# mbdriscoll/indigo

Measured on AMD Instinct MI355X. Metric: SENSE AHA evals/sec (256^3 x 8-coil non-Cartesian), higher is better.
Workload: dtype complex64 (f32)

## Files before the change

indigo_amd/csrc/ig_spmm.hip:

```cpp
#include "ig_spmm_common.h"
#include <hip/amd_detail/amd_hip_unsafe_atomics.h>
#include <algorithm>
#include <atomic>
#include <cstring>

namespace {

struct GridMask {
    const uint32_t* bits;
    int64_t n0, nm;
};

constexpr int WL_SUB = 32;
struct WorkLists {
    int32_t*  rows[2];
    uint32_t* count;
    uint32_t  cap;
    const int32_t* yperm;
};

__device__ __forceinline__ bool wl_append(const WorkLists& wl, int which, int sub, bool want, int32_t row) {
    const uint64_t bal = __ballot(want);
    if (!bal) return false;
    const int lane = threadIdx.x & 63;
    const int leader = __ffsll((long long)bal) - 1;
    uint32_t base = 0;
    if (lane == leader) base = atomicAdd(&wl.count[which * WL_SUB + sub], (uint32_t)__popcll(bal));
    base = __shfl(base, leader, 64);
    if (!want) return false;
    const uint32_t idx = base + (uint32_t)__popcll(bal & ((1ull << lane) - 1ull));
    if (idx >= wl.cap) return false;
    wl.rows[which][(size_t)sub * wl.cap + idx] = row;
    return true;
}

__device__ __forceinline__ int64_t out_row(const int32_t* __restrict__ perm, int64_t row) {
    return perm ? (int64_t)perm[row] : row;
}

template <bool CONJ>
__device__ __forceinline__ void acc_nz(float2& acc, float2 v, float2 x) {
    if (CONJ) acc = cadd(acc, cmulc(v, x));
    else      cfma(acc, v, x);
}

template <int CL, int NL, bool CONJ, int BMODE>
__global__ void __launch_bounds__(BLK)
k_csrmm_gather(int64_t M, int64_t N,
               const int32_t* __restrict__ rowptr, const int32_t* __restrict__ colind,
               const float2* __restrict__ vals,
               const float2* __restrict__ X, int64_t ldx, int64_t sxr,
               float2* __restrict__ Y, int64_t ldy,
               float2 alpha, float2 beta, int xcd_remap,
               WorkLists wl, int32_t thr_mid, int32_t thr_long) {
    constexpr int RPW = 64 / (CL * NL);
    const int lane = threadIdx.x & 63;
    const int c = lane % CL;
    const int i = (lane / CL) % NL;
    const int r = lane / (CL * NL);
    const int64_t blk = xcd_remap ? xcd_block(blockIdx.x, gridDim.x) : (int64_t)blockIdx.x;
    const int64_t wave = blk * WAVES_PER_BLOCK + (threadIdx.x >> 6);
    const int64_t row = wave * RPW + r;
    const bool row_ok = row < M;

    int32_t p0 = 0, p1 = 0;
    if (row_ok) { p0 = rowptr[row]; p1 = rowptr[row + 1]; }

    int deferred = 0;
    const int32_t len = p1 - p0;
    {
        const int sub = (int)(wave & (WL_SUB - 1));
        const bool head = c == 0 && i == 0;
        if (wl_append(wl, 0, sub, head && len > thr_mid && len <= thr_long, (int32_t)row)) deferred = 1;
        if (wl_append(wl, 1, sub, head && len > thr_long, (int32_t)row)) deferred = 1;
    }
    deferred = __shfl(deferred, r * CL * NL, 64);
    if (deferred) p1 = p0;

    for (int64_t jb = 0; jb < N; jb += CL) {
        const int64_t j = jb + c;
        const bool col_ok = j < N;
        const float2* __restrict__ xcol = X + (col_ok ? j : 0) * ldx;
        float2 acc = make_float2(0.f, 0.f);
        for (int32_t p = p0 + i; p < p1; p += 4 * NL) {
            int32_t k4[4];
            float2 v4[4], x4[4];
#pragma unroll
            for (int u = 0; u < 4; ++u) {
                const int32_t pu = p + u * NL;
                const bool ok = pu < p1;
                const int32_t q = ok ? pu : p1 - 1;
                k4[u] = colind[q];
                const float2 vv = vals[q];
                v4[u] = ok ? vv : make_float2(0.f, 0.f);
            }
#pragma unroll
            for (int u = 0; u < 4; ++u) x4[u] = xcol[k4[u] * sxr];
#pragma unroll
            for (int u = 0; u < 4; ++u) acc_nz<CONJ>(acc, v4[u], x4[u]);
        }
#pragma unroll
        for (int off = CL * NL / 2; off >= CL; off >>= 1) {
            acc.x += __shfl_xor(acc.x, off, 64);
            acc.y += __shfl_xor(acc.y, off, 64);
        }
        if (i == 0 && row_ok && col_ok && !deferred) {
            float2* yp = Y + j * ldy + out_row(wl.yperm, row);
            float2 out = cmul(alpha, acc);
            if (BMODE == 1) cfma(out, beta, *yp);
            *yp = out;
        }
    }
}

template <int VW, int CLV, int NL, bool CONJ, int BMODE, bool REALW = false>
__global__ void __launch_bounds__(BLK)
k_csrmm_gather_v(int64_t M, const int32_t* __restrict__ rowptr, const int32_t* __restrict__ colind,
                 const float2* __restrict__ vals, const float2* __restrict__ X, int64_t sxr,
                 float2* __restrict__ Y, int64_t ldy, float2 alpha, float2 beta, int xcd_remap,
                 WorkLists wl, int32_t thr_mid, int32_t thr_long) {
    static_assert(VW % 2 == 0 && CLV * NL <= 64, "16-byte loads; a row's lanes fit a wave");
    constexpr int LPR = CLV * NL, RPW = 64 / LPR, NV = VW / 2;
    const int lane = threadIdx.x & 63;
    const int c = lane % CLV, i = (lane / CLV) % NL, r = lane / LPR;
    const int64_t blk = xcd_remap ? xcd_block(blockIdx.x, gridDim.x) : (int64_t)blockIdx.x;
    const int64_t wave = blk * WAVES_PER_BLOCK + (threadIdx.x >> 6);
    const int64_t row = wave * RPW + r;
    const bool row_ok = row < M;
    int32_t p0 = 0, p1 = 0;
    if (row_ok) { p0 = rowptr[row]; p1 = rowptr[row + 1]; }
    int deferred = 0;
    const int32_t len = p1 - p0;
    {
        const int sub = (int)(wave & (WL_SUB - 1));
        const bool head = c == 0 && i == 0;
        if (wl_append(wl, 0, sub, head && len > thr_mid && len <= thr_long, (int32_t)row)) deferred = 1;
        if (wl_append(wl, 1, sub, head && len > thr_long, (int32_t)row)) deferred = 1;
    }
    deferred = __shfl(deferred, r * LPR, 64);
    if (deferred) p1 = p0;
    float2 acc[VW];
#pragma unroll
    for (int u = 0; u < VW; ++u) acc[u] = make_float2(0.f, 0.f);
    const float4* __restrict__ X4 = reinterpret_cast<const float4*>(X + c * VW);
    for (int32_t p = p0 + i; p < p1; p += 4 * NL) {
        int32_t k4[4];
        float2 v4[4];
        float4 x4[4][NV];
#pragma unroll
        for (int u = 0; u < 4; ++u) {
            const int32_t pu = p + u * NL;
            const bool ok = pu < p1;
            const int32_t q = ok ? pu : p1 - 1;
            k4[u] = colind[q];
            const float2 vv = REALW ? make_float2(reinterpret_cast<const float*>(vals)[q], 0.f) : vals[q];
            v4[u] = ok ? vv : make_float2(0.f, 0.f);
        }
#pragma unroll
        for (int u = 0; u < 4; ++u)
#pragma unroll
            for (int h = 0; h < NV; ++h) x4[u][h] = X4[((int64_t)k4[u] * sxr) / 2 + h];
#pragma unroll
        for (int u = 0; u < 4; ++u)
#pragma unroll
            for (int h = 0; h < NV; ++h) {
                if (REALW) {
                    acc[2 * h].x = fmaf(v4[u].x, x4[u][h].x, acc[2 * h].x);         acc[2 * h].y = fmaf(v4[u].x, x4[u][h].y, acc[2 * h].y);
                    acc[2 * h + 1].x = fmaf(v4[u].x, x4[u][h].z, acc[2 * h + 1].x); acc[2 * h + 1].y = fmaf(v4[u].x, x4[u][h].w, acc[2 * h + 1].y);
                } else {
                    acc_nz<CONJ>(acc[2 * h], v4[u], make_float2(x4[u][h].x, x4[u][h].y));
                    acc_nz<CONJ>(acc[2 * h + 1], v4[u], make_float2(x4[u][h].z, x4[u][h].w));
                }
            }
    }
#pragma unroll
    for (int off = LPR / 2; off >= CLV; off >>= 1)
#pragma unroll
        for (int u = 0; u < VW; ++u) {
            acc[u].x += __shfl_xor(acc[u].x, off, 64);
            acc[u].y += __shfl_xor(acc[u].y, off, 64);
        }
    if (i == 0 && row_ok && !deferred) {
        const int64_t orow = out_row(wl.yperm, row);
#pragma unroll
        for (int u = 0; u < VW; ++u) {
            float2* yp = Y + (int64_t)(c * VW + u) * ldy + orow;
            float2 out = cmul(alpha, acc[u]);
            if (BMODE == 1) cfma(out, beta, *yp);
            *yp = out;
        }
    }
}

template <bool CONJ, int BMODE, int NW >
__global__ void __launch_bounds__(64 * NW)
k_csrmm_gather_tile64(int64_t M, int64_t nnz, const int32_t* __restrict__ rowptr, const int32_t* __restrict__ colind,
                      const float2* __restrict__ vals, const float2* __restrict__ X ,
                      float2* __restrict__ Y, int64_t ldy, float2 alpha, float2 beta, int xcd_remap,
                      WorkLists wl, int32_t thr_long) {
    constexpr int TLD = 65, U = 7, RPW = 64 / NW;
    __shared__ float2 tile[64 * TLD];
    const int lane = threadIdx.x & 63, c = lane & 15, i = lane >> 4;
    const int wv = __builtin_amdgcn_readfirstlane(threadIdx.x >> 6);
    const int64_t blk = xcd_remap ? xcd_block(blockIdx.x, gridDim.x) : (int64_t)blockIdx.x;
    const int64_t row0 = blk * 64;
    if (row0 >= M) return;
    int32_t myp;
    {
        int64_t r = row0 + wv + NW * (lane >> 1) + (lane & 1);
        if (lane >= 2 * RPW || r > M) r = M;
        myp = rowptr[r];
    }
    const float4* __restrict__ X4 = reinterpret_cast<const float4*>(X) + c * 2;
    const int32_t last = (int32_t)(nnz - 1);
    auto load_raw = [&](int32_t a, int32_t b, int32_t& rk, float2& rv) {
        rk = 0; rv = make_float2(0.f, 0.f);
        if (lane < 4 * U) {
            const int32_t pu = a + lane;
            const bool ok = pu < b;
            int32_t q = ok ? pu : b - 1;
            q = q < 0 ? 0 : (q > last ? last : q);
            rk = colind[q];
            const float2 t = vals[q];
            rv = ok ? t : make_float2(0.f, 0.f);
        }
    };
    auto spread = [&](int32_t rk, float2 rv, int32_t (&kk)[U], float2 (&vv)[U]) {
#pragma unroll
        for (int u = 0; u < U; ++u) {
            const int src = (i + 4 * u) * 4;
            kk[u] = __builtin_amdgcn_ds_bpermute(src, rk);
            vv[u].x = __int_as_float(__builtin_amdgcn_ds_bpermute(src, __float_as_int(rv.x)));
            vv[u].y = __int_as_float(__builtin_amdgcn_ds_bpermute(src, __float_as_int(rv.y)));
        }
    };
    auto load_idx = [&](int32_t a, int32_t b, int32_t (&kk)[U], float2 (&vv)[U]) {
        int32_t rk; float2 rv;
        load_raw(a, b, rk, rv);
        spread(rk, rv, kk, vv);
    };
    auto gather = [&](const int32_t (&kk)[U], const float2 (&vv)[U], float2 (&acc)[4]) {
        float4 x4[U][2];
#pragma unroll
        for (int u = 0; u < U; ++u) {
            x4[u][0] = X4[(int64_t)kk[u] * 32];
            x4[u][1] = X4[(int64_t)kk[u] * 32 + 1];
        }
#pragma unroll
        for (int u = 0; u < U; ++u) {
            acc_nz<CONJ>(acc[0], vv[u], make_float2(x4[u][0].x, x4[u][0].y));
            acc_nz<CONJ>(acc[1], vv[u], make_float2(x4[u][0].z, x4[u][0].w));
            acc_nz<CONJ>(acc[2], vv[u], make_float2(x4[u][1].x, x4[u][1].y));
            acc_nz<CONJ>(acc[3], vv[u], make_float2(x4[u][1].z, x4[u][1].w));
        }
    };
    unsigned skip = 0;
    int32_t p0 = __builtin_amdgcn_readlane(myp, 0), p1 = __builtin_amdgcn_readlane(myp, 1);
    int32_t k[U];
    float2 v[U];
    load_idx(p0, p1, k, v);
#pragma unroll 1
    for (int j = 0; j < RPW; ++j) {
        const int jn = j + 1 < RPW ? j + 1 : RPW - 1;
        int32_t q0 = __builtin_amdgcn_readlane(myp, 2 * jn), q1 = __builtin_amdgcn_readlane(myp, 2 * jn + 1);
        if (j == RPW - 1) q1 = q0;
        const int64_t row = row0 + wv + NW * j;
        bool deferred = false;
        if (p1 - p0 > thr_long && row < M) {
            const bool mine = wl_append(wl, 1, (int)((blk * NW + wv) & (WL_SUB - 1)), lane == 0, (int32_t)row);
            deferred = __builtin_amdgcn_readfirstlane((int)mine) != 0;
        }
        if (deferred || row >= M) skip |= 1u << j;
        float2 acc[4];
#pragma unroll
        for (int u = 0; u < 4; ++u) acc[u] = make_float2(0.f, 0.f);
        int32_t rkn;
        float2 rvn;
        if (!deferred) {
            float4 x4[U][2];
#pragma unroll
            for (int u = 0; u < U; ++u) {
                x4[u][0] = X4[(int64_t)k[u] * 32];
                x4[u][1] = X4[(int64_t)k[u] * 32 + 1];
            }
            load_raw(q0, q1, rkn, rvn);
#pragma unroll
            for (int u = 0; u < U; ++u) {
                acc_nz<CONJ>(acc[0], v[u], make_float2(x4[u][0].x, x4[u][0].y));
                acc_nz<CONJ>(acc[1], v[u], make_float2(x4[u][0].z, x4[u][0].w));
                acc_nz<CONJ>(acc[2], v[u], make_float2(x4[u][1].x, x4[u][1].y));
                acc_nz<CONJ>(acc[3], v[u], make_float2(x4[u][1].z, x4[u][1].w));
            }
            for (int32_t pp = p0 + 4 * U; pp < p1; pp += 4 * U) {
                int32_t k2[U];
                float2 v2[U];
                load_idx(pp, p1, k2, v2);
                gather(k2, v2, acc);
            }
#pragma unroll
            for (int u = 0; u < 4; ++u) {
                acc[u].x += __shfl_xor(acc[u].x, 16, 64); acc[u].y += __shfl_xor(acc[u].y, 16, 64);
                acc[u].x += __shfl_xor(acc[u].x, 32, 64); acc[u].y += __shfl_xor(acc[u].y, 32, 64);
            }
        } else {
            load_raw(q0, q1, rkn, rvn);
        }
        if (i == 0) {
// ... 322 lines not shown
        constexpr int UT = 16;
        for (int j0 = 0; j0 < nb; j0 += UT) {
            int32_t kk[UT]; float2 vv[UT], xx[UT]; int rj[UT];
#pragma unroll
            for (int u = 0; u < UT; ++u) {
                const int j = j0 + u < nb ? j0 + u : nb - 1;
                kk[u] = __shfl(k_i, j, 64);
                vv[u] = make_float2(__shfl(v_i.x, j, 64), __shfl(v_i.y, j, 64));
                rj[u] = __shfl(r_i, j, 64);
                if (j0 + u >= nb) vv[u] = make_float2(0.f, 0.f);
            }
#pragma unroll
            for (int u = 0; u < UT; ++u) xx[u] = Xp[(int64_t)kk[u] * 64 + lane];
#pragma unroll
            for (int u = 0; u < UT; ++u) {
                if (rj[u] != cur) {
                    tile[wv * 16 + cur][lane] = acc;
                    acc = make_float2(0.f, 0.f);
                    cur = rj[u];
                }
                if (!((defmask >> rj[u]) & 1ull)) acc_nz<CONJ>(acc, vv[u], xx[u]);
            }
        }
    }
    tile[wv * 16 + cur][lane] = acc;
    __syncthreads();
    const int64_t orow = (int64_t)blockIdx.x * 64 + lane;
    if (orow < M && !skip[lane]) {
#pragma unroll 4
        for (int c = wv * 16; c < wv * 16 + 16; ++c) {
            float2* yp = Y + (int64_t)c * ldy + out_row(wl.yperm, orow);
            float2 out = cmul(alpha, tile[lane][c]);
            if (BMODE == 1) cfma(out, beta, *yp);
            *yp = out;
        }
    }
}


template <int CL, bool CONJ, int BMODE>
__global__ void __launch_bounds__(BLK)
k_csrmm_rows_wave(int64_t N, const int32_t* __restrict__ rowptr, const int32_t* __restrict__ colind,
                  const float2* __restrict__ vals, const float2* __restrict__ X, int64_t ldx, int64_t sxr,
                  float2* __restrict__ Y, int64_t ldy, int64_t syr, float2 alpha, float2 beta,
                  const int32_t* __restrict__ list, const uint32_t* __restrict__ count, uint32_t cap,
                  const int32_t* __restrict__ yperm) {
    constexpr int NLW = 64 / CL;
    const int lane = threadIdx.x & 63;
    const int c = lane % CL, i = lane / CL;
    const uint32_t gw = blockIdx.x * WAVES_PER_BLOCK + (threadIdx.x >> 6);
    const uint32_t sub = gw % WL_SUB, nwaves = gridDim.x * WAVES_PER_BLOCK / WL_SUB;
    uint32_t n = count[sub];
    if (n > cap) n = cap;
    list += (size_t)sub * cap;
    for (uint32_t e = gw / WL_SUB; e < n; e += nwaves) {
        const int64_t row = list[e];
        const int32_t p0 = rowptr[row], p1 = rowptr[row + 1];
        for (int64_t jb = 0; jb < N; jb += CL) {
            const int64_t j = jb + c;
            const bool col_ok = j < N;
            const float2* __restrict__ xcol = X + (col_ok ? j : 0) * ldx;
            float2 a0 = make_float2(0.f, 0.f), a1 = a0, a2 = a0, a3 = a0;
            int32_t p = p0 + i;
            for (; p + 3 * NLW < p1; p += 4 * NLW) {
                const int32_t k0 = colind[p], k1 = colind[p + NLW], k2 = colind[p + 2 * NLW], k3 = colind[p + 3 * NLW];
                const float2 v0 = vals[p], v1 = vals[p + NLW], v2 = vals[p + 2 * NLW], v3 = vals[p + 3 * NLW];
                const float2 x0 = xcol[k0 * sxr], x1 = xcol[k1 * sxr], x2 = xcol[k2 * sxr], x3 = xcol[k3 * sxr];
                acc_nz<CONJ>(a0, v0, x0); acc_nz<CONJ>(a1, v1, x1);
                acc_nz<CONJ>(a2, v2, x2); acc_nz<CONJ>(a3, v3, x3);
            }
            for (; p < p1; p += NLW) acc_nz<CONJ>(a0, vals[p], xcol[colind[p] * sxr]);
            float2 acc = cadd(cadd(a0, a1), cadd(a2, a3));
#pragma unroll
            for (int off = 32; off >= CL; off >>= 1) {
                acc.x += __shfl_xor(acc.x, off, 64);
                acc.y += __shfl_xor(acc.y, off, 64);
            }
            if (i == 0 && col_ok) {
                float2* yp = Y + j * ldy + out_row(yperm, row) * syr;
                float2 out = cmul(alpha, acc);
                if (BMODE == 1) cfma(out, beta, *yp);
                *yp = out;
            }
        }
    }
}

template <int CL, bool CONJ, int BMODE>
__global__ void __launch_bounds__(1024)
k_csrmm_rows_block(int64_t N, const int32_t* __restrict__ rowptr, const int32_t* __restrict__ colind,
                   const float2* __restrict__ vals, const float2* __restrict__ X, int64_t ldx, int64_t sxr,
                   float2* __restrict__ Y, int64_t ldy, int64_t syr, float2 alpha, float2 beta,
                   const int32_t* __restrict__ list, const uint32_t* __restrict__ count, uint32_t cap,
                   const int32_t* __restrict__ yperm) {
    constexpr int NLB = 1024 / CL;
    __shared__ float2 part[16][64];
    const int tid = threadIdx.x, lane = tid & 63, wid = tid >> 6;
    const int c = tid % CL, i = tid / CL;
    const uint32_t sub = blockIdx.x % WL_SUB, nblk = gridDim.x / WL_SUB;
    uint32_t n = count[sub];
    if (n > cap) n = cap;
    list += (size_t)sub * cap;
    for (uint32_t e = blockIdx.x / WL_SUB; e < n; e += nblk) {
        const int64_t row = list[e];
        const int32_t p0 = rowptr[row], p1 = rowptr[row + 1];
        for (int64_t jb = 0; jb < N; jb += CL) {
            const int64_t j = jb + c;
            const bool col_ok = j < N;
            const float2* __restrict__ xcol = X + (col_ok ? j : 0) * ldx;
            float2 a0 = make_float2(0.f, 0.f), a1 = a0, a2 = a0, a3 = a0;
            int32_t p = p0 + i;
            for (; p + 3 * NLB < p1; p += 4 * NLB) {
                const int32_t k0 = colind[p], k1 = colind[p + NLB], k2 = colind[p + 2 * NLB], k3 = colind[p + 3 * NLB];
                const float2 v0 = vals[p], v1 = vals[p + NLB], v2 = vals[p + 2 * NLB], v3 = vals[p + 3 * NLB];
                const float2 x0 = xcol[k0 * sxr], x1 = xcol[k1 * sxr], x2 = xcol[k2 * sxr], x3 = xcol[k3 * sxr];
                acc_nz<CONJ>(a0, v0, x0); acc_nz<CONJ>(a1, v1, x1);
                acc_nz<CONJ>(a2, v2, x2); acc_nz<CONJ>(a3, v3, x3);
            }
            for (; p < p1; p += NLB) acc_nz<CONJ>(a0, vals[p], xcol[colind[p] * sxr]);
            float2 acc = cadd(cadd(a0, a1), cadd(a2, a3));
#pragma unroll
            for (int off = 32; off >= CL; off >>= 1) {
                acc.x += __shfl_xor(acc.x, off, 64);
                acc.y += __shfl_xor(acc.y, off, 64);
            }
            part[wid][lane] = acc;
            __syncthreads();
            if (tid < CL) {
                float2 sum = make_float2(0.f, 0.f);
#pragma unroll
                for (int w = 0; w < 16; ++w) sum = cadd(sum, part[w][tid]);
                if (col_ok) {
                    float2* yp = Y + j * ldy + out_row(yperm, row) * syr;
                    float2 out = cmul(alpha, sum);
                    if (BMODE == 1) cfma(out, beta, *yp);
                    *yp = out;
                }
            }
            __syncthreads();
        }
    }
}

template <int CL, int NL, bool ATOMIC>
__global__ void __launch_bounds__(BLK)
k_csrmm_scatter(int64_t M, int64_t N,
                const int32_t* __restrict__ rowptr, const int32_t* __restrict__ colind,
                const float2* __restrict__ vals,
                const float2* __restrict__ X, int64_t ldx,
                float2* __restrict__ Y, int64_t ldy,
                float2 alpha, int xcd_remap) {
    constexpr int RPW = 64 / (CL * NL);
    const int lane = threadIdx.x & 63;
    const int c = lane % CL;
    const int i = (lane / CL) % NL;
    const int r = lane / (CL * NL);
    const int64_t blk = xcd_remap ? xcd_block(blockIdx.x, gridDim.x) : (int64_t)blockIdx.x;
    const int64_t wave = blk * WAVES_PER_BLOCK + (threadIdx.x >> 6);
    const int64_t row = wave * RPW + r;
    if (row >= M) return;
    const int32_t p0 = rowptr[row], p1 = rowptr[row + 1];
    if (p0 == p1) return;

    for (int64_t jb = 0; jb < N; jb += CL) {
        const int64_t j = jb + c;
        if (j >= N) continue;
        const float2 ax = cmul(alpha, X[j * ldx + row]);
        float2* __restrict__ ycol = Y + j * ldy;
        for (int32_t p = p0 + i; p < p1; p += NL) {
            const int32_t k = colind[p];
            const float2 t = cmulc(vals[p], ax);
            if (ATOMIC) {
                unsafeAtomicAdd(&ycol[k].x, t.x);
                unsafeAtomicAdd(&ycol[k].y, t.y);
            } else {
                float2 y = ycol[k];
                y.x += t.x; y.y += t.y;
                ycol[k] = y;
            }
        }
    }
}

template <bool ZERO>
__global__ void __launch_bounds__(BLK)
k_panel_scale(int64_t rows, int64_t N, float2* __restrict__ Y, int64_t ld, float2 beta) {
    const int64_t j = blockIdx.y;
    float2* __restrict__ col = Y + j * ld;
    for (int64_t k = (int64_t)blockIdx.x * BLK + threadIdx.x; k < rows; k += (int64_t)gridDim.x * BLK) {
        if (ZERO) col[k] = make_float2(0.f, 0.f);
        else      col[k] = cmul(beta, col[k]);
    }
}

template <int NP>
__global__ void __launch_bounds__(BLK)
k_pack_panel(int64_t rows, int64_t N, const float2* __restrict__ X, int64_t ld, float2* __restrict__ Xp,
             const int32_t* __restrict__ xperm) {
    for (int64_t e = (int64_t)blockIdx.x * BLK + threadIdx.x; e < rows * NP; e += (int64_t)gridDim.x * BLK) {
        const int64_t k = e / NP;
        const int c = (int)(e % NP);
        const int64_t src = xperm ? (int64_t)xperm[k] : k;
        Xp[e] = c < N ? X[c * ld + src] : make_float2(0.f, 0.f);
    }
}

template <int NP>
__global__ void __launch_bounds__(BLK)
k_pack_panel_tiled(int64_t rows, int64_t N, const float2* __restrict__ X, int64_t ld, float2* __restrict__ Xp,
                   const int32_t* __restrict__ xperm) {
    __shared__ float2 tile[NP][65];
    const int tid = threadIdx.x;
    const int kk = tid & 63, c0 = tid >> 6;
    constexpr int PER = NP / (BLK / 64);
    float2 v[PER];
    auto load = [&](int64_t k0) {
        const int64_t k = k0 + kk;
        const int64_t src = k < rows ? (xperm ? (int64_t)xperm[k] : k) : 0;
#pragma unroll
        for (int u = 0; u < PER; ++u) {
            const int c = c0 + u * (BLK / 64);
            v[u] = (c < N && k < rows) ? X[c * ld + src] : make_float2(0.f, 0.f);
        }
    };
    int64_t k0 = (int64_t)blockIdx.x * 64;
    if (k0 < rows) load(k0);
    for (; k0 < rows; k0 += (int64_t)gridDim.x * 64) {
#pragma unroll
        for (int u = 0; u < PER; ++u) tile[c0 + u * (BLK / 64)][kk] = v[u];
        __syncthreads();
        const int64_t kn = k0 + (int64_t)gridDim.x * 64;
        if (kn < rows) load(kn);
        for (int e = tid; e < 64 * NP; e += BLK) {
            const int r = e / NP, c = e % NP;
            if (k0 + r < rows) Xp[(k0 + r) * NP + c] = tile[c][r];
        }
        __syncthreads();
    }
}

}

int ig_pack_panel(ig_ctx* ctx, int64_t rows, int64_t N, int np, const float2* X, int64_t ldx, const int32_t* xperm,
                  bool may_decline, const float2** packed) {
    *packed = nullptr;
    const size_t need = (size_t)rows * np * 8;
    if (may_decline && (need == 0 || need > ((size_t)16 << 30))) return IG_OK;
    if (ctx->xpack_bytes < need) {
        if (may_decline) {
            size_t free_b = 0, total_b = 0;
            if (hipMemGetInfo(&free_b, &total_b) != hipSuccess) { (void)hipGetLastError(); free_b = 0; }
            if (need > (free_b + ctx->xpack_bytes) / 4) return IG_OK;
        }
        if (ctx->d_xpack) { IG_HIP(ctx, hipStreamSynchronize(ctx->stream)); IG_HIP(ctx, hipFree(ctx->d_xpack)); ctx->d_xpack = nullptr; ctx->xpack_bytes = 0; }
        if (!may_decline) {
            IG_HIP(ctx, hipMalloc((void**)&ctx->d_xpack, need));
        } else if (hipMalloc((void**)&ctx->d_xpack, need) != hipSuccess) { (void)hipGetLastError(); ctx->d_xpack = nullptr; return IG_OK; }
        ctx->xpack_bytes = need;
    }
    ig_prof_scope prof(ctx, "pack_panel", (double)rows * N * 8.0 + (double)need);
    float2* xp = (float2*)ctx->d_xpack;
    const int64_t cap = (int64_t)ctx->num_cu * 16;
    int64_t g = np <= 8 ? (rows * np + BLK - 1) / BLK : (rows + 63) / 64;
    if (g > cap) g = cap;
#define IG_PACK(KERNEL_) hipLaunchKernelGGL(KERNEL_, dim3((unsigned)g), dim3(BLK), 0, ctx->stream, rows, N, X, ldx, xp, xperm)
    if (np == 1)       IG_PACK(k_pack_panel<1>);
    else if (np == 2)  IG_PACK(k_pack_panel<2>);
    else if (np == 4)  IG_PACK(k_pack_panel<4>);
    else if (np == 8)  IG_PACK(k_pack_panel<8>);
    else if (np == 16) IG_PACK(k_pack_panel_tiled<16>);
    else if (np == 32) IG_PACK(k_pack_panel_tiled<32>);
    else               IG_PACK(k_pack_panel_tiled<64>);
#undef IG_PACK
    IG_LAUNCH_CHECK(ctx, "k_pack_panel");
    *packed = xp;
    return IG_OK;
}

namespace {


template <int NC, int NSEG , bool PAIR = false, bool REALW = false>
__global__ void __launch_bounds__(BLK)
k_grid_bricks(const BrickTask* __restrict__ tasks, int ntasks, const BrickRef* __restrict__ btab,
              const BrickEntry* __restrict__ entries , const uint32_t* __restrict__ round_rows,
              const float2* __restrict__ Xp ,
              float2* __restrict__ Y, float2 alpha, const uint32_t* __restrict__ bits,
              int n0, int nm, int bm_log2, int bs_log2, int nbx, int nbm, int st_log2 , int zw ) {
    extern __shared__ float2 acc_all[];
    constexpr int TPR = 64 / NC;
    constexpr int RS = 64 / TPR;
    const int tid = threadIdx.x, lane = tid & 63;
    const int wv = __builtin_amdgcn_readfirstlane(tid >> 6);
    const int task = blockIdx.x * WAVES_PER_BLOCK + wv;
    if (task >= ntasks) return;
    const BrickTask tk = tasks[task];
    const int nb = tk.nb_flags & 0xffff;
    const bool shared = (tk.nb_flags >> 16) & 1;
    const int32_t nent = tk.hi - tk.lo, nround = nent / TPR;
    const int xs_log2 = 4 - st_log2, seg_log2 = xs_log2 + bm_log2 + bs_log2;
    const int BM = 1 << bm_log2, nseg = NSEG ? (PAIR ? 2 * NSEG : NSEG) : 1 << seg_log2, ncell = 16 << (bm_log2 + bs_log2);
    float2* __restrict__ acc = acc_all + (size_t)wv * ncell * NC;
    const int coil = lane % NC, tsub = lane / NC, xround = (lane / NC) % RS;
    const rsrc_t r_en = REALW ? make_rsrc(reinterpret_cast<const float2*>(entries) + tk.lo) : make_rsrc(entries + tk.lo);
    const rsrc_t r_rr = make_rsrc(round_rows + tk.lo / TPR), r_x = make_rsrc(Xp);

    struct Set { u3 en; uint32_t rid; float2 x; };
    Set s0, s1, s2, s3;
    auto request_samples = [&](Set& s, int st) {
        const int32_t q = st * RS + xround;
        s.rid = (uint32_t)buf_ld_i32(r_rr, q < nround ? (unsigned)q * 4u : IG_OOB);
    };
    auto request_entries = [&](Set& s, int st) {
        const int32_t idx = st * 64 + lane;
        if (REALW) {
            const float2 t = buf_ld<false>(r_en, idx < nent ? (unsigned)idx * 8u : IG_OOB, 0);
            s.en.x = __float_as_uint(t.x); s.en.y = __float_as_uint(t.y); s.en.z = 0u;
        } else {
            s.en = buf_ld_u3(r_en, idx < nent ? (unsigned)idx * 12u : IG_OOB);
        }
    };
    auto request_rows = [&](Set& s, int st) {
        const int32_t q = st * RS + xround;
        s.x = buf_ld<false>(r_x, q < nround ? (s.rid * (unsigned)NC + (unsigned)coil) * 8u : IG_OOB, 0);
    };
    request_samples(s0, 0);
    request_samples(s1, 1);
    const float2 my_ref = buf_ld<false>(make_rsrc(btab + tk.bt), lane < nb ? (unsigned)lane * 8u : IG_OOB, 0);
    request_entries(s0, 0);
    request_samples(s2, 2);
    request_samples(s3, 3);
    request_entries(s1, 1);
    request_entries(s2, 2);
    request_rows(s0, 0);
    request_samples(s0, 4);
    request_rows(s1, 1);
    int my_end = 0x7fffffff, my_pt = 0, my_bx = 0, my_m0 = 0, my_s0 = 0;
    if (lane < nb) {
        const int brick = (int)__float_as_uint(my_ref.x);
        if (!shared) my_end = (int)__float_as_uint(my_ref.y) - tk.lo;
        my_bx = brick % nbx;
        my_m0 = ((brick / nbx) % nbm) << bm_log2;
        my_s0 = (brick / (nbx * nbm)) << bs_log2;
        my_pt = my_bx * 16 + n0 * (my_m0 + nm * my_s0);
    }
    uint32_t my_mask = 0xffffffffu;
    if (bits) {
        const int nt = n0 >> st_log2;
        const rsrc_t r_bits = make_rsrc(bits);
        uint32_t w[8];
#pragma unroll
        for (int p = 0; p < 8; ++p) {
            const int pair = p * 64 + lane, j = pair >> seg_log2, seg = pair & (nseg - 1);
            const int jbx = __shfl(my_bx, j & 63), jm0 = __shfl(my_m0, j & 63), js0 = __shfl(my_s0, j & 63);
            const int xs = seg & ((1 << xs_log2) - 1), im = (seg >> xs_log2) & (BM - 1), is = seg >> (xs_log2 + bm_log2);
            const int km = jm0 + im, ks = js0 + is;
            const int kmq = km / zw, kmr = km - kmq * zw;
            w[p] = (uint32_t)buf_ld_i32(r_bits, j < nb ? (unsigned)((ks * nt + (jbx << xs_log2) + xs) * zw + kmr) * 4u : IG_OOB) >> kmq;
        }
        my_mask = 0u;
#pragma unroll
        for (int p = 0; p < 8; ++p) {
            const uint64_t bal = __ballot(w[p] & 1u);
            const int first = (p * 64) >> seg_log2, per = 64 >> seg_log2;
            if (lane >= first && lane < first + per)
                my_mask = (uint32_t)(bal >> ((lane - first) << seg_log2)) & (nseg == 32 ? 0xffffffffu : (1u << nseg) - 1u);
        }
    }
    for (int e = lane; e < ncell * NC; e += 64) acc[e] = make_float2(0.f, 0.f);

    int cur = 0;
    int32_t cur_end = __builtin_amdgcn_readlane(my_end, 0);
    auto flush_segment = [&](int pt, uint32_t mask, int seg) {
        const uint32_t flags = PAIR ? (mask >> (2 * seg)) & 3u : (mask >> seg) & 1u;
        if (!flags) return;
        const bool mine = PAIR ? ((flags >> (lane >> 5)) & 1u) != 0 : true;
        const int f_log2 = PAIR ? 3 : st_log2, fx_log2 = 4 - f_log2;
        const int xs = seg & ((1 << fx_log2) - 1), im = (seg >> fx_log2) & (BM - 1), is = seg >> (fx_log2 + bm_log2);
        const int cell0 = (xs << f_log2) + 16 * (im + BM * is);
        float2* src = acc + (size_t)cell0 * NC;
        float2* dst = Y + ((int64_t)pt + (xs << f_log2) + (int64_t)n0 * (im + (int64_t)nm * is)) * NC;
        const int nel = NC << f_log2;
        for (int e = lane; e < nel; e += 64) {
            const float2 o = cmul(alpha, src[e]);
            if (mine) {
                if (shared) {
                    asm volatile("global_atomic_add_f32 %0, %1, off\n\tglobal_atomic_add_f32 %0, %2, off offset:4"
                                 :: "v"(dst + e), "v"(o.x), "v"(o.y) : "memory");
                } else {
                    asm volatile("global_store_dwordx2 %0, %1, off" :: "v"(dst + e), "v"(o) : "memory");
                }
            }
            src[e] = make_float2(0.f, 0.f);
        }
    };
    auto flush = [&]() {
        const int pt = __builtin_amdgcn_readlane(my_pt, cur);
        const uint32_t mask = (uint32_t)__builtin_amdgcn_readlane((int)my_mask, cur);
        if (NSEG) {
#pragma unroll
            for (int seg = 0; seg < (NSEG ? NSEG : 1); ++seg) flush_segment(pt, mask, seg);
        } else {
            for (int seg = 0; seg < nseg; ++seg) flush_segment(pt, mask, seg);
        }
        ++cur;
        cur_end = __builtin_amdgcn_readlane(my_end, cur & 63);
    };
    auto super_trip = [&](const Set& s, Set& next, Set& rows_ahead, Set& entries_ahead, int st) {
        const uint32_t e_cell = s.en.x, e_re = s.en.y, e_im = s.en.z;
        const float x_re = s.x.x, x_im = s.x.y;
        request_rows(rows_ahead, st + 2);
        request_entries(entries_ahead, st + 3);
        request_samples(next, st + 5);
        for (int r = 0; r < RS; ++r) {
            const int32_t start = st * 64 + r * TPR;
            if (start >= nent) break;
            if (start >= cur_end) flush();
            const int from_e = (r * TPR + tsub) * 4, from_x = (r * NC + coil) * 4;
            const uint32_t cell = (uint32_t)__builtin_amdgcn_ds_bpermute(from_e, (int)e_cell);
            const float vr = __int_as_float(__builtin_amdgcn_ds_bpermute(from_e, (int)e_re));
            const float vi = REALW ? 0.f : __int_as_float(__builtin_amdgcn_ds_bpermute(from_e, (int)e_im));
            const float xr = __int_as_float(__builtin_amdgcn_ds_bpermute(from_x, __float_as_int(x_re)));
            const float xi = __int_as_float(__builtin_amdgcn_ds_bpermute(from_x, __float_as_int(x_im)));
            if (cell != 0xffffffffu) {
                float2* a = acc + (int)cell * NC + coil;
                float2 v = *a;
                if (REALW) {
                    v.x = fmaf(vr, xr, v.x);
                    v.y = fmaf(vr, xi, v.y);
                } else {
                    v.x += fmaf(vr, xr, vi * xi);
                    v.y += fmaf(vr, xi, -vi * xr);
                }
                *a = v;
            }
        }
    };
    const int nst = (nent + 63) / 64;
    for (int st = 0; st < nst; st += 4) {
        super_trip(s0, s1, s2, s3, st);
        super_trip(s1, s2, s3, s0, st + 1);
        super_trip(s2, s3, s0, s1, st + 2);
        super_trip(s3, s0, s1, s2, st + 3);
    }
    flush();
}

struct SlotEntry { uint32_t cell; float re, im; uint32_t row; };

template <int NC, bool REALW = false>
__global__ void __launch_bounds__(BLK)
k_grid_slots(const BrickTask* __restrict__ tasks, int ntasks, const BrickRef* __restrict__ btab,
             const int32_t* __restrict__ slot_ptr, const SlotEntry* __restrict__ entries,
             const float2* __restrict__ Xp , float2* __restrict__ Y, float2 alpha,
             const uint32_t* __restrict__ bits, int n0, int nm, int bm_log2, int bs_log2, int nbx, int nbm, int st_log2, int zw ) {
    extern __shared__ float2 acc_all[];
    const int tid = threadIdx.x, lane = tid & 63;
    const int wv = __builtin_amdgcn_readfirstlane(tid >> 6);
    const int task = blockIdx.x * WAVES_PER_BLOCK + wv;
    if (task >= ntasks) return;
    const BrickTask tk = tasks[task];
    const int nb = tk.nb_flags & 0xffff;
    const bool shared = (tk.nb_flags >> 16) & 1;
    const int32_t nslot = tk.hi - tk.lo;
    const int xs_log2 = 4 - st_log2, seg_log2 = xs_log2 + bm_log2 + bs_log2;
    const int BM = 1 << bm_log2, nseg = 1 << seg_log2, ncell = 16 << (bm_log2 + bs_log2);
    float2* __restrict__ acc = acc_all + (size_t)wv * ncell * NC;
    const float2 my_ref = buf_ld<false>(make_rsrc(btab + tk.bt), lane < nb ? (unsigned)lane * 8u : IG_OOB, 0);
    int my_end = 0x7fffffff, my_pt = 0, my_bx = 0, my_m0 = 0, my_s0 = 0;
    if (lane < nb) {
        const int brick = (int)__float_as_uint(my_ref.x);
        if (!shared) my_end = (int)__float_as_uint(my_ref.y) - tk.lo;
        my_bx = brick % nbx;
        my_m0 = ((brick / nbx) % nbm) << bm_log2;
        my_s0 = (brick / (nbx * nbm)) << bs_log2;
        my_pt = my_bx * 16 + n0 * (my_m0 + nm * my_s0);
    }
    uint32_t my_mask = 0xffffffffu;
    if (bits) {
        const int nt = n0 >> st_log2;
        const rsrc_t r_bits = make_rsrc(bits);
        uint32_t w[8];
#pragma unroll
        for (int p = 0; p < 8; ++p) {
            const int pair = p * 64 + lane, j = pair >> seg_log2, seg = pair & (nseg - 1);
            const int jbx = __shfl(my_bx, j & 63), jm0 = __shfl(my_m0, j & 63), js0 = __shfl(my_s0, j & 63);
            const int xs = seg & ((1 << xs_log2) - 1), im = (seg >> xs_log2) & (BM - 1), is = seg >> (xs_log2 + bm_log2);
            const int km = jm0 + im, ks = js0 + is;
            const int kmq = km / zw, kmr = km - kmq * zw;
            w[p] = (uint32_t)buf_ld_i32(r_bits, j < nb ? (unsigned)((ks * nt + (jbx << xs_log2) + xs) * zw + kmr) * 4u : IG_OOB) >> kmq;
        }
        my_mask = 0u;
#pragma unroll
        for (int p = 0; p < 8; ++p) {
            const uint64_t bal = __ballot(w[p] & 1u);
            const int first = (p * 64) >> seg_log2, per = 64 >> seg_log2;
            if (lane >= first && lane < first + per)
                my_mask = (uint32_t)(bal >> ((lane - first) << seg_log2)) & (nseg == 32 ? 0xffffffffu : (1u << nseg) - 1u);
        }
    }
    for (int e = lane; e < ncell * NC; e += 64) acc[e] = make_float2(0.f, 0.f);

    int cur = 0;
    int32_t cur_end = __builtin_amdgcn_readlane(my_end, 0);
    auto flush = [&]() {
        __builtin_amdgcn_fence(__ATOMIC_RELEASE, "wavefront");
        __builtin_amdgcn_wave_barrier();
        __builtin_amdgcn_fence(__ATOMIC_ACQUIRE, "wavefront");
        const int pt = __builtin_amdgcn_readlane(my_pt, cur);
        const uint32_t mask = (uint32_t)__builtin_amdgcn_readlane((int)my_mask, cur);
        for (int seg = 0; seg < nseg; ++seg) {
            if (!((mask >> seg) & 1u)) continue;
            const int xs = seg & ((1 << xs_log2) - 1), im = (seg >> xs_log2) & (BM - 1), is = seg >> (xs_log2 + bm_log2);
            const int cell0 = (xs << st_log2) + 16 * (im + BM * is);
            float2* src = acc + (size_t)cell0 * NC;
            float2* dst = Y + ((int64_t)pt + (xs << st_log2) + (int64_t)n0 * (im + (int64_t)nm * is)) * NC;
            const int nel = NC << st_log2;
            for (int e = lane; e < nel; e += 64) {
                const float2 o = cmul(alpha, src[e]);
                if (shared) {
                    asm volatile("global_atomic_add_f32 %0, %1, off\n\tglobal_atomic_add_f32 %0, %2, off offset:4"
                                 :: "v"(dst + e), "v"(o.x), "v"(o.y) : "memory");
                } else {
                    asm volatile("global_store_dwordx2 %0, %1, off" :: "v"(dst + e), "v"(o) : "memory");
                }
                src[e] = make_float2(0.f, 0.f);
            }
        }
        ++cur;
        cur_end = __builtin_amdgcn_readlane(my_end, cur & 63);
    };

    const rsrc_t r_sp = make_rsrc(slot_ptr + tk.lo), r_en = make_rsrc(entries), r_x = make_rsrc(Xp);
    struct XV { float2 v[NC]; };
    auto load_entry = [&](int32_t off, int32_t n) -> SlotEntry {
        SlotEntry e;
        if (REALW) {
            const u3 q = buf_ld_u3(r_en, lane < n ? (unsigned)(off + lane) * 12u : IG_OOB);
            e.cell = lane < n ? q.x : 0xffffffffu; e.re = __uint_as_float(q.y); e.im = 0.f; e.row = q.z;
        } else {
            const float4 q = buf_ld_f4(r_en, lane < n ? (unsigned)(off + lane) * 16u : IG_OOB);
            e.cell = lane < n ? __float_as_uint(q.x) : 0xffffffffu; e.re = q.y; e.im = q.z; e.row = __float_as_uint(q.w);
        }
        return e;
    };
    auto load_x = [&](const SlotEntry& e) -> XV {
        XV x;
        const unsigned o = e.cell != 0xffffffffu ? e.row * (unsigned)(NC * 8) : IG_OOB;
        if (NC == 1) x.v[0] = buf_ld<false>(r_x, o, 0);
        else {
#pragma unroll
            for (int c = 0; c < NC; c += 2) {
                const float4 q = buf_ld_f4(r_x, o == IG_OOB ? IG_OOB : o + (unsigned)c * 8u);
                x.v[c] = make_float2(q.x, q.y); x.v[c + 1] = make_float2(q.z, q.w);
            }
        }
        return x;
    };
    for (int32_t base = 0; base < nslot; base += 63) {
        const int32_t left = nslot - base, cnt = left < 63 ? left : 63;
        const int32_t sp = buf_ld_i32(r_sp, lane <= cnt ? (unsigned)(base + lane) * 4u : IG_OOB);
        auto slot_off = [&](int i) { return __builtin_amdgcn_readlane(sp, i); };
        SlotEntry e0 = load_entry(slot_off(0), slot_off(1) - slot_off(0));
        SlotEntry e1 = cnt > 1 ? load_entry(slot_off(1), slot_off(2) - slot_off(1)) : SlotEntry{0xffffffffu, 0.f, 0.f, 0u};
        XV x0 = load_x(e0);
#pragma unroll 1
        for (int i = 0; i < cnt; ++i) {
            SlotEntry e2{0xffffffffu, 0.f, 0.f, 0u};
            if (i + 2 < cnt) e2 = load_entry(slot_off(i + 2), slot_off(i + 3) - slot_off(i + 2));
            const XV x1 = load_x(e1);
            if (base + i >= cur_end) flush();
            if (e0.cell != 0xffffffffu) {
#pragma unroll
                for (int c = 0; c < NC; ++c) {
                    float2* a = acc + (int)e0.cell * NC + c;
                    float2 t = *a;
                    if (REALW) {
                        t.x = fmaf(e0.re, x0.v[c].x, t.x);
                        t.y = fmaf(e0.re, x0.v[c].y, t.y);
                    } else {
                        t.x += fmaf(e0.re, x0.v[c].x, e0.im * x0.v[c].y);
                        t.y += fmaf(e0.re, x0.v[c].y, -e0.im * x0.v[c].x);
                    }
                    *a = t;
                }
            }
            e0 = e1; e1 = e2; x0 = x1;
        }
    }
    flush();
}

template <int NC>
__global__ void __launch_bounds__(BLK)
k_grid_bricks_zero(const int32_t* __restrict__ shared_bricks, float2* __restrict__ Y, const uint32_t* __restrict__ bits,
                   int n0, int nm, int bm_log2, int bs_log2, int nbx, int nbm, int st_log2, int zw) {
    const int brick = shared_bricks[blockIdx.x];
    const int xs_log2 = 4 - st_log2;
    const int BM = 1 << bm_log2, nseg = 1 << (xs_log2 + bm_log2 + bs_log2);
    const int bx = brick % nbx, bmi = (brick / nbx) % nbm, bsi = brick / (nbx * nbm);
    const int x0 = bx * 16, m0 = bmi << bm_log2, s0 = bsi << bs_log2;
    const int nt = n0 >> st_log2, lane = threadIdx.x & 63, wv = threadIdx.x >> 6;
    for (int seg = wv; seg < nseg; seg += WAVES_PER_BLOCK) {
        const int xs = seg & ((1 << xs_log2) - 1), im = (seg >> xs_log2) & (BM - 1), is = seg >> (xs_log2 + bm_log2);
        const int km = m0 + im, ks = s0 + is;
        if (bits && !((bits[((size_t)ks * nt + (bx << xs_log2) + xs) * zw + (km % zw)] >> (km / zw)) & 1u)) continue;
        float2* dst = Y + ((int64_t)x0 + (xs << st_log2) + (int64_t)n0 * (km + (int64_t)nm * ks)) * NC;
        for (int e = lane; e < (NC << st_log2); e += 64) dst[e] = make_float2(0.f, 0.f);
    }
}

inline int pow2_ceil(int64_t v, int cap) {
    int p = 1;
    while (p < v && p < cap) p <<= 1;
    return p;
}

struct Shape { int CL, NL; };

inline Shape pick_shape(int64_t rows, int64_t N, int64_t nnz) {
    Shape s;
    s.CL = pow2_ceil(N, 64);
    const int64_t mean = rows > 0 ? (nnz + rows - 1) / rows : 1;
    constexpr int nl_cap = 8;
    int cap = 64 / s.CL;
    if (nl_cap > 0 && mean <= 4 * nl_cap && cap > nl_cap) cap = nl_cap;
    s.NL = pow2_ceil(mean > 0 ? mean : 1, cap);
    return s;
}

constexpr uint32_t WL_CAP = 1u << 20;

int ensure_worklists(ig_ctx* ctx) {
    if (ctx->d_worklist) return IG_OK;
    const size_t bytes = sizeof(int32_t) * 2 * WL_CAP + 2 * WL_SUB * sizeof(uint32_t);
    IG_HIP(ctx, hipMalloc((void**)&ctx->d_worklist, bytes));
    ctx->worklist_bytes = bytes;
    return IG_OK;
}

template <bool CONJ>
int launch_gather(ig_ctx* ctx, int64_t rows, int64_t xrows, int64_t N, int64_t nnz,
                  const int32_t* rowptr, const int32_t* colind, const float2* vals,
                  const float2* X, int64_t ldx, float2* Y, int64_t ldy, float2 alpha, float2 beta,
                  GridMask mask = GridMask{nullptr, 0, 0}, const int32_t* yperm = nullptr,
                  const int32_t* xperm = nullptr, bool x_il = false, bool y_il = false, const float* rvals = nullptr) {
    const Shape s = pick_shape(rows, N, nnz);
    const int64_t syr = y_il ? N : 1;
    if (y_il) ldy = 1;
    int64_t sxc = ldx, sxr = 1;
    bool packed = false;
    if (x_il) { sxc = 1; sxr = N; packed = (N & (N - 1)) == 0 && N >= 1; }
    if (!x_il && N == 1 && !xperm) { sxc = ldx; sxr = 1; packed = true; }
    if (!x_il && ((N >= 2 && N <= 64 && nnz >= xrows) || (xperm && N <= 64))) {
        const int np = s.CL;
        const float2* xp = nullptr;
        if (int rc = ig_pack_panel(ctx, xrows, N, np, X, ldx, xperm, true, &xp)) return rc;
        if (xp) { X = xp; sxc = 1; sxr = np; packed = true; }
    }
    IG_REQUIRE(ctx, !xperm || packed, "csrmm: a panel-row list needs the packed path (2..64 columns and room for the repacked panel: a quarter of the free device memory, at most 16 GiB)");
    const int rpw = 64 / (s.CL * s.NL);
    const int64_t waves = (rows + rpw - 1) / rpw;
    const int64_t blocks = (waves + WAVES_PER_BLOCK - 1) / WAVES_PER_BLOCK;
    IG_REQUIRE(ctx, blocks <= 0x7fffffffLL, "csrmm: matrix too large for one launch (%lld blocks)", (long long)blocks);
    const int xcd = 1;
    const bool b0 = (beta.x == 0.f && beta.y == 0.f);

    const bool defer = true;
    const int nlw = 64 / s.CL;
    const int32_t thr_long = defer ? 256 * nlw : 0x7fffffff;
    const int32_t thr_mid = !defer ? 0x7fffffff : (nlw > s.NL ? 16 * s.NL : thr_long);
    WorkLists wl{};
    wl.yperm = yperm;
    if (defer) {
        if (int rc = ensure_worklists(ctx)) return rc;
        wl.rows[0] = ctx->d_worklist;
        wl.rows[1] = ctx->d_worklist + WL_CAP;
        wl.count = reinterpret_cast<uint32_t*>(ctx->d_worklist + 2 * WL_CAP);
        wl.cap = WL_CAP / WL_SUB;
        IG_HIP(ctx, hipMemsetAsync(wl.count, 0, 2 * WL_SUB * sizeof(uint32_t), ctx->stream));
    }
    constexpr int vw = 4;
    const bool wide_v = vw > 0 && packed && sxc == 1 && N == sxr && (N == 64 || N == 32 || N == 16) && !y_il &&
                        nnz >= 8 * rows && (reinterpret_cast<uintptr_t>(X) & 15u) == 0;
    const bool rowlane = !wide_v && (nnz <= 2 * rows || (packed && N >= 16 && nnz <= 8 * rows));
    if (rowlane) {
        ig_prof_scope prof(ctx, CONJ ? "csrmm_rowlane_conj" : "csrmm_rowlane");
        const int64_t rblocks = (rows + BLK - 1) / BLK;
        const int32_t tm_want = nnz <= 2 * rows ? 16 : 512;
        const int32_t tm = defer ? (thr_long < tm_want ? thr_long : tm_want) : 0x7fffffff;
#define IG_ROWLANE_L(NC_, BM_, PK_, U_, BUF_)                                                      \
    hipLaunchKernelGGL((k_csrmm_rowlane<NC_, CONJ, BM_, PK_, U_, BUF_>), dim3((unsigned)rblocks),  \
                       dim3(BLK), 0, ctx->stream, rows, N, rowptr, colind, vals, X, sxc, sxr, Y, ldy, \
                       alpha, beta, xcd, wl, tm, thr_long, mask)
#define IG_ROWLANE(NC_)                                                                            \
    do {                                                                                           \
        if (packed && b0 && NC_ >= 2 && bufok) {                                                   \
            IG_ROWLANE_L(NC_, 0, true, 2, true);                       \
        } else if (packed && b0) IG_ROWLANE_L(NC_, 0, true, 1, false);                             \
        else if (packed) IG_ROWLANE_L(NC_, 1, true, 1, false);                                     \
        else if (b0) IG_ROWLANE_L(NC_, 0, false, 1, false);                                        \
        else IG_ROWLANE_L(NC_, 1, false, 1, false);                                                \
    } while (0)
        const bool bufok = packed && nnz * 8 < 0x7fffffffLL && xrows * sxr * 8 < 0x7fffffffLL;
        constexpr int dense_thr = 32;
        if (packed && sxc == 1 && N == 64 && sxr == 64 && !y_il && !mask.bits) {
            const int64_t tblocks = (rows + 63) / 64;
            IG_REQUIRE(ctx, tblocks <= 0x7fffffffLL, "csrmm: matrix too large for one launch");
            const int32_t tt = defer ? (thr_long < 512 ? thr_long : 512) : 0x7fffffff;
            with_flag(!b0, [&](auto bmode) {
                hipLaunchKernelGGL((k_csrmm_rowtile64<CONJ, bmode>), dim3((unsigned)tblocks), dim3(BLK), 0, ctx->stream,
                                   rows, rowptr, colind, vals, X, Y, ldy, alpha, beta, wl, tt, thr_long); });
        } else
        if (dense_thr > 0 && packed && b0 && bufok && nnz <= 2 * rows && N == sxr && (sxr == 8 || sxr == 4 || sxr == 2 || sxr == 1)) {
            const int32_t td = defer ? (thr_long < dense_thr ? thr_long : dense_thr) : 0x7fffffff;
            int64_t dblocks = ((rows + 63) / 64 + WAVES_PER_BLOCK - 1) / WAVES_PER_BLOCK;
            IG_REQUIRE(ctx, dblocks <= 0x7fffffffLL, "csrmm: matrix too large for one launch");
#define IG_DENSE(NC_) with_flag(y_il, [&](auto yil) {                                                                              \
                hipLaunchKernelGGL((k_csrmm_dense64<NC_, CONJ, yil>), dim3((unsigned)dblocks), dim3(BLK), 0, ctx->stream,           \
                                   rows, rowptr, colind, vals, X, Y, ldy, alpha, wl, td, thr_long, mask, dense_co); })
            constexpr int dense_co = 1;
            if (sxr == 8) IG_DENSE(8); else if (sxr == 4) IG_DENSE(4); else if (sxr == 2) IG_DENSE(2);
            else hipLaunchKernelGGL((k_csrmm_dense64<1, CONJ, false>), dim3((unsigned)dblocks), dim3(BLK), 0, ctx->stream,
                                    rows, rowptr, colind, vals, X, Y, ldy, alpha, wl, td, thr_long, mask, dense_co);
#undef IG_DENSE
        } else if (y_il) {
            return ig_fail(ctx, IG_ERR_UNSUPPORTED, "csrmm: an interleaved result panel needs the dense-lane kernel (2, 4 or 8 columns, beta = 0)");
        } else
        if (s.CL >= 8) IG_ROWLANE(8);
        else if (s.CL == 4) IG_ROWLANE(4);
        else if (s.CL == 2) IG_ROWLANE(2);
        else IG_ROWLANE(1);
#undef IG_ROWLANE
#undef IG_ROWLANE_L
        IG_LAUNCH_CHECK(ctx, "k_csrmm_rowlane");
    } else {
        IG_REQUIRE(ctx, !y_il, "csrmm: an interleaved result panel is only supported for matrices with mostly empty rows");
// ... 654 lines not shown
```

Measured before the change: 163.3.

## Replace ds_bpermute broadcasts with DPP and permlane swaps for 8-coil grid kernel

```diff
diff --git a/indigo_amd/csrc/ig_spmm.hip b/indigo_amd/csrc/ig_spmm.hip
--- a/indigo_amd/csrc/ig_spmm.hip
+++ b/indigo_amd/csrc/ig_spmm.hip
@@ -3,6 +3,7 @@
 #include <algorithm>
 #include <atomic>
 #include <cstring>
+#include <type_traits>
 
 namespace {
 
@@ -931,6 +932,8 @@
     const int BM = 1 << bm_log2, nseg = NSEG ? (PAIR ? 2 * NSEG : NSEG) : 1 << seg_log2, ncell = 16 << (bm_log2 + bs_log2);
     float2* __restrict__ acc = acc_all + (size_t)wv * ncell * NC;
     const int coil = lane % NC, tsub = lane / NC, xround = (lane / NC) % RS;
+    constexpr bool REGS = NC == 8;
+    const int eslot = REGS ? ((lane & 15) >> 1) * 8 + 2 * (lane >> 4) + (lane & 1) : lane;
     const rsrc_t r_en = REALW ? make_rsrc(reinterpret_cast<const float2*>(entries) + tk.lo) : make_rsrc(entries + tk.lo);
     const rsrc_t r_rr = make_rsrc(round_rows + tk.lo / TPR), r_x = make_rsrc(Xp);
 
@@ -941,7 +944,7 @@
         s.rid = (uint32_t)buf_ld_i32(r_rr, q < nround ? (unsigned)q * 4u : IG_OOB);
     };
     auto request_entries = [&](Set& s, int st) {
-        const int32_t idx = st * 64 + lane;
+        const int32_t idx = st * 64 + eslot;
         if (REALW) {
             const float2 t = buf_ld<false>(r_en, idx < nent ? (unsigned)idx * 8u : IG_OOB, 0);
             s.en.x = __float_as_uint(t.x); s.en.y = __float_as_uint(t.y); s.en.z = 0u;
@@ -1041,16 +1044,7 @@
         request_rows(rows_ahead, st + 2);
         request_entries(entries_ahead, st + 3);
         request_samples(next, st + 5);
-        for (int r = 0; r < RS; ++r) {
-            const int32_t start = st * 64 + r * TPR;
-            if (start >= nent) break;
-            if (start >= cur_end) flush();
-            const int from_e = (r * TPR + tsub) * 4, from_x = (r * NC + coil) * 4;
-            const uint32_t cell = (uint32_t)__builtin_amdgcn_ds_bpermute(from_e, (int)e_cell);
-            const float vr = __int_as_float(__builtin_amdgcn_ds_bpermute(from_e, (int)e_re));
-            const float vi = REALW ? 0.f : __int_as_float(__builtin_amdgcn_ds_bpermute(from_e, (int)e_im));
-            const float xr = __int_as_float(__builtin_amdgcn_ds_bpermute(from_x, __float_as_int(x_re)));
-            const float xi = __int_as_float(__builtin_amdgcn_ds_bpermute(from_x, __float_as_int(x_im)));
+        auto accumulate = [&](uint32_t cell, float vr, float vi, float xr, float xi) {
             if (cell != 0xffffffffu) {
                 float2* a = acc + (int)cell * NC + coil;
                 float2 v = *a;
@@ -1062,6 +1056,56 @@
                     v.y += fmaf(vr, xi, -vi * xr);
                 }
                 *a = v;
+            }
+        };
+        if constexpr (REGS) {
+            int ur[4], ui[4];
+            {
+                const unsigned wr = __float_as_uint(x_re), wi = __float_as_uint(x_im);
+                const auto hr = __builtin_amdgcn_permlane32_swap(wr, wr, false, false);
+                const auto hi = __builtin_amdgcn_permlane32_swap(wi, wi, false, false);
+                const auto r01 = __builtin_amdgcn_permlane16_swap(hr[0], hr[0], false, false), r23 = __builtin_amdgcn_permlane16_swap(hr[1], hr[1], false, false);
+                const auto i01 = __builtin_amdgcn_permlane16_swap(hi[0], hi[0], false, false), i23 = __builtin_amdgcn_permlane16_swap(hi[1], hi[1], false, false);
+                ur[0] = (int)r01[0]; ur[1] = (int)r01[1]; ur[2] = (int)r23[0]; ur[3] = (int)r23[1];
+                ui[0] = (int)i01[0]; ui[1] = (int)i01[1]; ui[2] = (int)i23[0]; ui[3] = (int)i23[1];
+            }
+            int ec = (int)e_cell, ew = (int)e_re, ez = (int)e_im;
+            auto round = [&](int start, auto half) -> bool {
+                constexpr int H = decltype(half)::value;
+                if (start >= nent) return false;
+                if (start >= cur_end) flush();
+                constexpr int LO = 0x150 + 2 * H, HI = 0x151 + 2 * H;
+                const uint32_t cell = (uint32_t)__builtin_amdgcn_update_dpp(__builtin_amdgcn_mov_dpp(ec, LO, 0xf, 0x3, false), ec, HI, 0xf, 0xc, false);
+                const float vr = __int_as_float(__builtin_amdgcn_update_dpp(__builtin_amdgcn_mov_dpp(ew, LO, 0xf, 0x3, false), ew, HI, 0xf, 0xc, false));
+                const float vi = REALW ? 0.f : __int_as_float(__builtin_amdgcn_update_dpp(__builtin_amdgcn_mov_dpp(ez, LO, 0xf, 0x3, false), ez, HI, 0xf, 0xc, false));
+                const float xr = __int_as_float(__builtin_amdgcn_update_dpp(ur[0], ur[0], 0x128, 0xf, H ? 0x3 : 0xc, false));
+                const float xi = __int_as_float(__builtin_amdgcn_update_dpp(ui[0], ui[0], 0x128, 0xf, H ? 0x3 : 0xc, false));
+                accumulate(cell, vr, vi, xr, xi);
+                return true;
+            };
+#pragma unroll 1
+            for (int p = 0; p < RS / 2; ++p) {
+                const int32_t start = st * 64 + p * 2 * TPR;
+                if (!round(start, std::integral_constant<int, 0>())) break;
+                if (!round(start + TPR, std::integral_constant<int, 1>())) break;
+                ec = __builtin_amdgcn_mov_dpp(ec, 0x12c, 0xf, 0xf, false);
+                ew = __builtin_amdgcn_mov_dpp(ew, 0x12c, 0xf, 0xf, false);
+                if (!REALW) ez = __builtin_amdgcn_mov_dpp(ez, 0x12c, 0xf, 0xf, false);
+                ur[0] = ur[1]; ur[1] = ur[2]; ur[2] = ur[3];
+                ui[0] = ui[1]; ui[1] = ui[2]; ui[2] = ui[3];
+            }
+        } else {
+            for (int r = 0; r < RS; ++r) {
+                const int32_t start = st * 64 + r * TPR;
+                if (start >= nent) break;
+                if (start >= cur_end) flush();
+                const int from_e = (r * TPR + tsub) * 4, from_x = (r * NC + coil) * 4;
+                const uint32_t cell = (uint32_t)__builtin_amdgcn_ds_bpermute(from_e, (int)e_cell);
+                const float vr = __int_as_float(__builtin_amdgcn_ds_bpermute(from_e, (int)e_re));
+                const float vi = REALW ? 0.f : __int_as_float(__builtin_amdgcn_ds_bpermute(from_e, (int)e_im));
+                const float xr = __int_as_float(__builtin_amdgcn_ds_bpermute(from_x, __float_as_int(x_re)));
+                const float xi = __int_as_float(__builtin_amdgcn_ds_bpermute(from_x, __float_as_int(x_im)));
+                accumulate(cell, vr, vi, xr, xi);
             }
         }
     };
```

New measurement: 168.5 (median of 6 runs). 3.2% higher.
